# MaartenGr/ReinLife

Measured on AMD Instinct MI355X. Metric: agent-steps/sec (env.step + policy fwd), 30x30 grid, 100 agents, higher is better.
Workload: dtype f32-grade policy via block-scaled 2 x f16 split on v_mfma_f32_32x32x16_f16 (f32 accumulate) / int32+u8 world state / f64 rewards

## Files before the change

### reinlife_amd/csrc/rl_run.hip

```cpp
#include <mutex>
#include "rl_world_dev.h"
#ifndef RL_XM_DUELING_KERNEL
#define RL_XM_DUELING_KERNEL 0
#endif
#if RL_XM_DUELING_KERNEL != 0 && !defined(RL_XM_SELF_GENERATED_STATES_ONLY)
#error "RL_XM_DUELING_KERNEL != 0 is valid for self-generated states only: add -DRL_XM_SELF_GENERATED_STATES_ONLY to an A/B build that knows"
#endif
#ifndef RL_XM_ALL_DUELING_TILE
#define RL_XM_ALL_DUELING_TILE RL_XM_ALL_KERNEL
#endif
#ifndef RL_CERT_ALL
#define RL_CERT_ALL 0
#endif
#ifndef RL_XM_ALL_KERNEL
#define RL_XM_ALL_KERNEL 2
#endif

#ifdef RL_TUNING
#if !(defined(RL_RUN_UNIT) && RL_RUN_UNIT == 1)
static int g_run_debug = 0;
extern "C" __attribute__((visibility("default"))) void rl_debug_set_run_mask(int mask) { g_run_debug = mask; }
extern "C" __attribute__((visibility("default"))) int rl_debug_get_run_mask(void) { return g_run_debug; }
#endif
#define RL_RUN_DBG(ka) (*(const int __attribute__((address_space(4)))*)&(ka)->ra.debug)
static __device__ unsigned long long g_cert_counts[4];
#define RL_CERT_COUNT(greedy_mask, cert_mask, fell_back) do { \
        const unsigned long long gm_ = (greedy_mask), cm_ = (cert_mask); const bool fb_ = (fell_back); \
        if (__builtin_amdgcn_mbcnt_hi(~0u, __builtin_amdgcn_mbcnt_lo(~0u, 0u)) == 0) { \
            atomicAdd(&g_cert_counts[0], (unsigned long long)__popcll(gm_)); atomicAdd(&g_cert_counts[1], (unsigned long long)__popcll(cm_)); \
            if (fb_) atomicAdd(&g_cert_counts[2], 1ull); } } while (0)
#else
#define RL_RUN_DBG(ka) 0
#endif
#ifdef RL_TUNING
#if defined(RL_RUN_UNIT) && RL_RUN_UNIT == 1
extern "C" __attribute__((visibility("default"))) int rl_debug_cert_counters_all(unsigned long long* out)
#else
extern "C" __attribute__((visibility("default"))) int rl_debug_cert_counters(unsigned long long* out)
#endif
{
    const unsigned long long zero[4] = {0, 0, 0, 0};
    if (hipDeviceSynchronize() != hipSuccess || hipMemcpyFromSymbol(out, HIP_SYMBOL(g_cert_counts), sizeof(zero)) != hipSuccess) return -1;
    return hipMemcpyToSymbol(HIP_SYMBOL(g_cert_counts), zero, sizeof(zero)) == hipSuccess ? 0 : -1;
}
#endif

namespace {

#include "rl_policy_dev.h"

constexpr int kRunMaxBrains = 8;
constexpr int kKindAll = 4;
__host__ __device__ constexpr int kind_widest(int KIND) { return KIND == kKindAll ? RL_PPO : KIND; }

#ifndef RL_RUN_COHERENT
#define RL_RUN_COHERENT true
#endif
struct RunArgs {
    const float* packed[kRunMaxBrains];
    float eps[kRunMaxBrains];
    int kind[kRunMaxBrains];
    float* obs[2];
    int first;
    int n_ticks;
    int8_t* actions;
    const float* eps_sched;
    int eps_inline_on;
    float eps_inline[RL_EPS_INLINE_MAX];
    int trk_skip;
    int capture;
    float* policy_out;
    rl_replay rp[kRunMaxBrains];
    int debug;
};

struct PolSmem {
    short* prow;
    int* bstart;
    int* bcnt;
    int* tstart;
    short* trow;
    int* tbrain;
    int* meta;
    float* pairv;
    float* cconst;
    float* xmirror;
    int xrows;
    int xbytes;
    double* trk_scr;
    TrkLds trk;
    int* wtask;
    int* texoff;
    int* bkind;
    int* oflags;
};
constexpr int kMaxTiles = 32;
constexpr int kPairFloats = 32 + 2 * 64;
constexpr int kPairExBytes = 8 * kPlanes * 64 * 16;
constexpr int kPairFloatsAll = kPairValFloats + 2 * 64;
template <int KIND> __host__ __device__ constexpr int run_const_floats() { return KIND == kKindAll ? kTileConstMax : kTileConstFloats + kTileCertFloats; }
static_assert(kTileConstFloats + kTileCertFloats <= kTileConstMax, "kKindAll: the dueling block's value bound fits behind its constants");
template <int KIND> __host__ __device__ constexpr int run_pair_floats() { return KIND == kKindAll ? kPairFloatsAll : kPairFloats; }
template <int KIND>
__host__ __device__ inline size_t carve_policy(PolSmem& ps, char* base, size_t o, int cap, size_t mirror_budget = 0, int n_cbrains = 0,
                                               int pair_floats = run_pair_floats<KIND>(),
                                               size_t min_region = 0)
{
    o = align16(o);
    ps.xmirror = nullptr; ps.xrows = 0; ps.xbytes = 0;
    const size_t tail = 10 * (size_t)cap + 5120 + sizeof(float) * 4 * (size_t)pair_floats + sizeof(float) * run_const_floats<KIND>() * (size_t)n_cbrains;
    if (mirror_budget > o + tail) {
        const size_t rows = (mirror_budget - o - tail) / (sizeof(float) * kXStride);
        ps.xrows = (int)(rows < (size_t)cap ? rows : (size_t)cap);
        if (ps.xrows >= 32) {
            size_t bytes = sizeof(float) * kXStride * (size_t)ps.xrows;
            if (bytes < min_region && o + tail + min_region <= mirror_budget) bytes = min_region;
            ps.xmirror = (float*)(base + o); ps.xbytes = (int)bytes; o = align16(o + bytes);
        } else ps.xrows = 0;
    }
    ps.prow = (short*)(base + o); o = align16(o + sizeof(short) * (size_t)cap);
    ps.bstart = (int*)(base + o); o = align16(o + sizeof(int) * 64);
    ps.bcnt = (int*)(base + o); o = align16(o + sizeof(int) * 64);
    ps.tstart = (int*)(base + o); o = align16(o + sizeof(int) * 64);
    ps.trow = (short*)(base + o); o = align16(o + sizeof(short) * kMaxTiles * 32);
    ps.tbrain = (int*)(base + o); o = align16(o + sizeof(int) * kMaxTiles);
    ps.meta = (int*)(base + o); o = align16(o + sizeof(int) * 16);
    ps.cconst = nullptr;
    if (n_cbrains > 0) { ps.cconst = (float*)(base + o); o = align16(o + sizeof(float) * run_const_floats<KIND>() * (size_t)n_cbrains); }
    ps.pairv = nullptr;
    if (n_cbrains > 0) { ps.pairv = (float*)(base + o); o = align16(o + sizeof(float) * 4 * (size_t)pair_floats); }
    ps.wtask = (int*)(base + o); o = align16(o + sizeof(int) * 8);
    ps.texoff = (int*)(base + o); o = align16(o + sizeof(int) * 4);
    ps.bkind = (int*)(base + o); o = align16(o + sizeof(int) * kRunMaxBrains);
    if (KIND == kKindAll) { ps.oflags = (int*)(base + o); o = align16(o + sizeof(int) * 4); }
    else ps.oflags = nullptr;
    ps.trk_scr = (double*)(base + o); o = align16(o + sizeof(double) * (size_t)cap);
    ps.trk.sum = (double*)(base + o); o = align16(o + sizeof(double) * kRunMaxBrains * RL_TRK_VARS);
    ps.trk.pop = (double*)(base + o); o = align16(o + sizeof(double) * 2);
    ps.trk.cnt = (int*)(base + o); o = align16(o + sizeof(int) * kRunMaxBrains * RL_TRK_VARS);
    return o;
}
struct RunParams;
typedef const RunParams __attribute__((address_space(4))) RunParamsC;

struct RecycleRegs {
    unsigned short pos;
    int h, age, ma, g, b, u;
    uint8_t fl;
    signed char act;
    double f;
};
__device__ inline RecycleRegs recycle_read(Smem& s, int n)
{
    const int tid = rl_tidx();
    const int a = tid < n ? s.order[tid] : 0;
    RecycleRegs r;
    r.pos = s.pos[a];
    r.h = s.health[a]; r.age = s.age[a]; r.ma = s.max_age[a]; r.g = s.gene[a]; r.b = s.brain[a]; r.u = s.uid[a];
    r.fl = s.flags[a];
    r.act = s.action[a];
    r.f = s.fitness[a];
    return r;
}
#ifndef RL_SEAM_OPEN
#define RL_SEAM_OPEN 1
#endif
template <int T, bool SPEC>
__device__ __forceinline__ void recycle_world(const KParams& p, Smem& s, int n, int tick, int epoch, int next_uid, int max_gene, bool drain_stores, const RecycleRegs& rr,
                                              const int* also_drain = nullptr,
                                              bool open = false)
{
    const int tid = rl_tidx();
    const bool mine = tid < n;
    const unsigned short r_pos = rr.pos;
    const int r_h = rr.h, r_age = rr.age, r_ma = rr.ma, r_g = rr.g, r_b = rr.b, r_u = rr.u;
    const uint8_t r_fl = rr.fl;
    const signed char r_act = rr.act;
    const double r_f = rr.f;
    lds_barrier();
    if (mine) {
        s.pos[tid] = r_pos; s.health[tid] = r_h; s.age[tid] = r_age; s.max_age[tid] = r_ma; s.gene[tid] = r_g; s.brain[tid] = r_b;
        s.uid[tid] = r_u; s.flags[tid] = r_fl; s.fitness[tid] = r_f;
        if (!open) s.action[tid] = r_act;
        s.aux[tid] = 0; s.src[tid] = (short)tid; s.order[tid] = (short)tid; s.newidx[tid] = (short)tid;
        s.occ[(r_pos & 255) * p.W + (r_pos >> 8)] = (short)tid;
    }
    for (int c = tid; c < p.Cp; c += T) ((unsigned*)s.foodv)[c] = 0u;
    for (int i = tid; i < p.hash_size; i += T) { s.hkey[i] = -1; s.hcnt[i] = 0u; }
    if (tid < RL_MAX_BRAINS) s.present[tid] = 0;
    if (SPEC) for (int i = tid; i < 2 * p.cap; i += T) ((unsigned*)s.reward)[i] = 0u;
    if (tid < S_COUNT)
        s.scal[tid] = tid == S_NSLOTS ? n : tid == S_TICK ? tick : tid == S_EPOCH ? epoch : tid == S_NEXT_UID ? next_uid : tid == S_MAX_GENE ? max_gene : 0;
    const bool drain = drain_stores || (also_drain && __builtin_amdgcn_readfirstlane(*also_drain) != 0);
    if (drain) asm volatile("s_waitcnt vmcnt(0)" ::: "memory");
    if (!open || drain) lds_barrier();
}

struct RunParams {
    KParams p;
    RunArgs ra;
};
template <int TRAIN>
__device__ inline float run_eps(RunParamsC* ka, int b, int n_brains, const PolSmem& ps)
{
    typedef const float __attribute__((address_space(4))) cfloat;
    if (TRAIN) {
        if (*(const int __attribute__((address_space(4)))*)&ka->ra.eps_inline_on)
            return ((cfloat*)ka->ra.eps_inline)[__builtin_amdgcn_readfirstlane(ps.meta[3]) * n_brains + b];
        const float* es = *(const float* const __attribute__((address_space(4)))*)&ka->ra.eps_sched;
        if (es) return ((cfloat*)es)[__builtin_amdgcn_readfirstlane(ps.meta[3]) * n_brains + b];
    }
    return ((cfloat*)ka->ra.eps)[b];
}

__host__ __device__ constexpr int run_plane_stride(int T, int W, int H) { return T >= 512 ? plane_stride(W, H) : W; }
template <bool FIXED, int T>
__device__ inline KParams run_params(RunParamsC* ka)
{
#if defined(__HIP_DEVICE_COMPILE__)
    KParams p = *(const KParams __attribute__((address_space(4)))*)&ka->p;
#else
    KParams p{};
#endif
    if (FIXED) {
        p.W = kFixW; p.H = kFixH; p.C = kFixC; p.Cp = kFixCp; p.nW = kFixCp / 64; p.PS = run_plane_stride(T, kFixW, kFixH); p.invW = kFixInvW;
        p.cap = kFixCap; p.hash_size = kFixHash; p.hash_mask = kFixHash - 1;
    }
    return p;
}
constexpr size_t kRunLdsBudget = 160 * 1024;
__host__ __device__ constexpr size_t run_mirror_budget(int T) { return T >= 512 ? kRunLdsBudget : 0; }
__host__ __device__ constexpr int run_cbrains(int T, int n_brains) { return T >= 512 ? n_brains : 0; }
template <int KIND> __host__ __device__ constexpr int run_tile_floats(int T) { return T == 1024 ? kQuadFloats : run_pair_floats<KIND>(); }
__host__ __device__ constexpr size_t run_min_region(int T) { return T == 1024 ? 4 * (size_t)kQuadExBytes : 0; }
template <bool FIXED, int KIND>
__device__ inline void run_carve(const KParams& p, Smem& s, PolSmem& ps, char* smem_raw, int T)
{
    const size_t o0 = FIXED ? carve(s, smem_raw, kFixCp, kFixCap, kFixHash, plane_words(run_plane_stride(T, kFixW, kFixH), kFixH, kFixCp))
                            : carve(s, smem_raw, p.Cp, p.cap, p.hash_size, plane_words(p.PS, p.H, p.Cp));
    carve_policy<KIND>(ps, smem_raw, o0, p.cap, run_mirror_budget(T), run_cbrains(T, p.n_brains), run_tile_floats<KIND>(T), run_min_region(T));
}

template <typename F>
__device__ inline void policy_lists_wave0(const KParams& p, PolSmem& ps, int n, int lane, F brain_of)
{
    if (lane < p.n_brains) ps.bcnt[lane] = 0;
    for (int base = 0; base < n; base += 64) {
        const int k = base + lane;
        if (k < n) {
            const int b = brain_of(k);
            const int pos = __hip_atomic_fetch_add(&ps.bcnt[b], 1, __ATOMIC_RELAXED, __HIP_MEMORY_SCOPE_WORKGROUP);
            ps.prow[k] = (short)(unsigned short)(pos | (b << 10));
        }
    }
    const int mine = lane < p.n_brains ? ps.bcnt[lane] : 0;
    const int tiles = (mine + 31) >> 5;
    const int tincl = wave_incl_scan(tiles);
    const int first_tile = tincl - tiles;
    if (lane < p.n_brains) ps.tstart[lane] = first_tile;
    if (lane == 63) ps.meta[0] = tincl;
    const int tt = min(read_lane(tincl, 63), kMaxTiles);
    for (int e = lane; e < tt * 32; e += 64) ps.trow[e] = (short)0x8000;
    if (lane < tt) {
        int b = 0;
        for (int bb = 1; bb < p.n_brains; ++bb) if (read_lane(first_tile, bb) <= lane && read_lane(mine, bb) > 0) b = bb;
        ps.tbrain[lane] = b;
    }
    for (int base = 0; base < n; base += 64) {
        const int k = base + lane;
        if (k < n) {
            const int e = (unsigned short)ps.prow[k], pos = e & 1023, b = e >> 10;
            const int t = ps.tstart[b] + (pos >> 5);
            if (t < kMaxTiles) ps.trow[t * 32 + (pos & 31)] = (short)k;
        }
    }
}

__device__ inline int run_obs_flags(const KParams& p, const Smem& s, int n, int bad_health)
{
    if (bad_health || n >= 2 * p.max_agents) return 0;
    return RL_XF_SCALE | (s.type[0] == RL_AGENT ? 0 : RL_XF_INT_HEALTH);
}

__device__ inline void policy_schedule_wave0(const KParams& p, PolSmem& ps, RunParamsC* ka, int lane, bool first_call = false)
{
    const int nt = __builtin_amdgcn_readfirstlane(ps.meta[0]);
    const int t = lane & 3;
    const int brain = ps.tbrain[t] & (kRunMaxBrains - 1);
    const int kind = ps.bkind[brain];
    const int cost = t < nt ? (kind == RL_PPO ? 672 : kind == RL_DQN ? 180 : 360) : 0;
    const int ex = t < nt ? pair_ex_bytes(kind) : 0;
    int rank = 0, off = 0, total_ex = 0;
#pragma unroll
    for (int u = 0; u < 4; ++u) {
        const int cu = __builtin_amdgcn_readlane(cost, u), eu = __builtin_amdgcn_readlane(ex, u);
        rank += (cu > cost || (cu == cost && u < t)) ? 1 : 0;
        off += u < t ? eu : 0;
        total_ex += eu;
    }
    const size_t mirror_bytes = (size_t)ps.xrows * kXStride * sizeof(float);
    const bool pair_ok = nt <= 4 && ps.xmirror != nullptr && ps.pairv != nullptr && (size_t)total_ex <= mirror_bytes;
    const int fit = (int)(mirror_bytes / (size_t)pair_ex_bytes(RL_PPO));
    const int want = (0x22331100 >> (4 * (lane & 7))) & 15;
    int tile = -1, tb = 0, tk = 0;
#pragma unroll
    for (int u = 0; u < 4; ++u) {
        const int bu = __builtin_amdgcn_readlane(brain, u), ku = __builtin_amdgcn_readlane(kind, u);
        if (u < nt && __builtin_amdgcn_readlane(rank, u) == want) { tile = u; tb = bu; tk = ku; }
    }
    if (lane < 4) ps.texoff[lane] = off;
    if (lane < 8) ps.wtask[lane] = (pair_ok && tile >= 0) ? (tile | ((lane & 1) << 8) | (tb << 12) | (tk << 20)) : -1;
    if (lane == 0) {
        ps.meta[5] = pair_ok ? 0 : 1;
        if (first_call) ps.meta[6] = fit < 1 ? 1 : (fit > 4 ? 4 : fit);
    }
}

template <int T, int KIND, int TRAIN>
__device__ __forceinline__ void run_policy1(const KParams& p, Smem& s, PolSmem& ps, RunParamsC* ka, int w, int n, const float* obs_rows, char* smem_base, int wave)
{
    const int lane = rl_lane_fresh(), j = lane & 31;
    [[maybe_unused]] const int tid = wave * 64 + lane;
#ifdef RL_PHASE_PROFILE
    const long long t_entry = (long long)clock64();
#endif
    int ntiles = __builtin_amdgcn_readfirstlane(ps.meta[0]);
    {
        const int dbg = RL_RUN_DBG(ka);
        if (dbg & 4) ntiles = min(ntiles, 2);
        if (dbg & 8) ntiles = min(ntiles, 1);
        if (dbg & 16) ntiles = min(ntiles, 3);
    }
    const bool mirrored = ps.xmirror != nullptr && __builtin_amdgcn_readfirstlane(ps.meta[4]) != 0;
    [[maybe_unused]] const bool cert = T == 512 && TRAIN != 2 && !(RL_RUN_DBG(ka) & 64);
    auto tile_io = [&](int ti, TileIO& io, int j) {
        const int b = __builtin_amdgcn_readfirstlane(ps.tbrain[ti]);
        const int e = (unsigned short)ps.trow[ti * 32 + j], k = e & 0x7fff;
        io.packed = (gfloat*)((const float* const __attribute__((address_space(4)))*)ka->ra.packed)[b];
        io.obs = obs_rows;
        io.row = (int64_t)w * p.cap + k;
        io.valid = !(e & 0x8000);
        io.eps = run_eps<TRAIN>(ka, b, p.n_brains, ps);
        io.out = TRAIN == 2 ? *(float* const __attribute__((address_space(4)))*)&ka->ra.policy_out : nullptr;
        io.actions = *(int8_t* const __attribute__((address_space(4)))*)&ka->ra.actions;
        io.seed = p.seed;
        io.key_world = (uint32_t)(p.world_base + w); io.key_tick = (uint32_t)s.scal[S_TICK]; io.key_epoch = (uint32_t)s.scal[S_EPOCH];
        io.key_index = (uint32_t)k;
        io.lds_actions_off = (int)((char*)s.action - smem_base); io.lds_slot = k;
        io.x_lds_off = (mirrored && k < ps.xrows) ? (int)((char*)(ps.xmirror + k * kXStride) - smem_base) : -1;
        io.c_lds_off = ps.cconst ? (int)((char*)(ps.cconst + run_const_floats<KIND>() * b) - smem_base) : -1;
#ifdef RL_PHASE_PROFILE
        io.prof = (p.prof && (int)blockIdx.x == p.prof_world && wave == 0) ? p.prof : nullptr;
        if (io.prof && lane == 0) { io.prof[100] = t_entry; io.prof[110] = (long long)clock64(); }
#endif
    };
    if constexpr (T == 1024) {
        const int q = __builtin_amdgcn_readfirstlane(wave >> 2), slot = wave & 3;
        for (int t0 = 0; t0 < ntiles; t0 += 4) {
            const int lane = rl_lane_fresh(), j = lane & 31;
            const int ti = t0 + slot;
            const bool have = ti < ntiles;
            TileIO io;
            Tile1Part part;
            QuadLds ql;
            ql.pmax = ps.pairv + kQuadFloats * slot; ql.val = ql.pmax + 3 * 32 * 4;
            ql.ex = (f32x4*)((char*)ps.xmirror + (size_t)kQuadExBytes * slot);
#ifdef RL_PHASE_PROFILE
            ql.prof = (p.prof && (int)blockIdx.x == p.prof_world && slot == 0) ? p.prof : nullptr;
#endif
            if (have) {
                tile_io(ti, io, j);
                if (ntiles > 4) io.x_lds_off = -1;
                policy_quad<KIND, RL_RUN_COHERENT>(io, lane, q, &ql, &part);
            } else {
#pragma unroll
                for (int i = 0; i < kQuadBarriers; ++i) lds_barrier();
            }
            lds_barrier();
            if (have && q == 0) tile1_finish<KIND>(io, lane, part.head, ql.val[j], part.draw, *(const f32x4*)((const float*)(smem_base + io.c_lds_off) + 768 + 8 + 4 * (lane >> 5)));
        }
    } else
    if (T == 512 && !cert && ps.pairv != nullptr && ntiles <= 4 && (size_t)ps.xrows * kXStride * sizeof(float) >= 4 * (size_t)kPairExBytes) {
        const int role = __builtin_amdgcn_readfirstlane(wave >> 2), slot = wave & 3;
        const bool have = slot < ntiles;
        TileIO io;
        Tile1Part part;
        PairLds pl;
        pl.val = ps.pairv + kPairFloats * slot; pl.pmax = pl.val + 32;
        pl.ex = (f32x4*)((char*)ps.xmirror + (size_t)kPairExBytes * slot);
        if (have) {
            tile_io(slot, io, j);
            policy_tile1s<KIND, RL_RUN_COHERENT, true, RL_XM_DUELING_KERNEL>(io, lane, role, &pl, &part);
        } else { lds_barrier(); lds_barrier(); }
#ifdef RL_PHASE_PROFILE
        if (p.prof && (int)blockIdx.x == p.prof_world && lane == 0) p.prof[116 + wave] = (long long)clock64();
#endif
        lds_barrier();
        if (have && role == 0) {
            const int fl = rl_lane_fresh();
            tile1_finish<KIND>(io, fl, part.head, pl.val[fl & 31], part.draw, *(const f32x4*)((const float*)(smem_base + io.c_lds_off) + 768 + 8 + 4 * (fl >> 5)));
        }
    } else {
        for (int ti = wave; ti < ntiles; ti += T / 64) {
            TileIO io;
            tile_io(ti, io, j);
            if (T == 512 && cert) policy_tile1s<KIND, RL_RUN_COHERENT, false, RL_XM_DUELING_KERNEL, T == 512 && TRAIN != 2>(io, lane);
            else if (T == 512) policy_tile1s<KIND, RL_RUN_COHERENT, false, RL_XM_DUELING_KERNEL>(io, lane);
            else policy_tile1<KIND, RL_RUN_COHERENT, true>(io, lane);
        }
#ifdef RL_PHASE_PROFILE
        if (T == 512 && p.prof && (int)blockIdx.x == p.prof_world && lane == 0) p.prof[116 + wave] = (long long)clock64();
#endif
    }
#ifdef RL_PHASE_PROFILE
    if (p.prof && (int)blockIdx.x == p.prof_world && tid == 0) p.prof[111] = (long long)clock64();
#endif
    lds_barrier();
#ifdef RL_PHASE_PROFILE
    if (p.prof && (int)blockIdx.x == p.prof_world && tid == 0) p.prof[112] = (long long)clock64();
#endif
}

#ifndef RL_XM_COLD_CALL
#define RL_XM_COLD_CALL 0
#endif
#ifndef RL_XM_LIKELY
#define RL_XM_LIKELY 1
#endif
#if RL_XM_LIKELY
#define RL_XM_EXPECT(x) __builtin_expect_with_probability(!!(x), 1, 0.9)
#else
#define RL_XM_EXPECT(x) (x)
#endif
template <bool CERT>
__device__ __attribute__((noinline, cold)) Tile1Part run_tile_general(TileIO io, PairLds pl, int role, int kind)
{
    Tile1Part part;
    const int lane = rl_lane_fresh();
    if (kind == RL_DQN) policy_pair2<RL_DQN, RL_RUN_COHERENT>(io, lane, role, &pl, &part);
    else if (kind == RL_PPO) policy_pair2<RL_PPO, RL_RUN_COHERENT>(io, lane, role, &pl, &part);
    else policy_tile1s<RL_PERD3QN, RL_RUN_COHERENT, true, 0, CERT>(io, lane, role, &pl, &part);
    return part;
}

template <int T, int TRAIN>
__device__ __forceinline__ void run_policy_all(const KParams& p, Smem& s, PolSmem& ps, RunParamsC* ka, int w, int n, const float* obs_rows, char* smem_base, int wave)
{
    static_assert(T == 512, "kKindAll: 512-thread workgroups");
    typedef const int __attribute__((address_space(4))) cint;
    const int lane = rl_lane_fresh(), j = lane & 31;
#ifdef RL_PHASE_PROFILE
    if (p.prof && (int)blockIdx.x == p.prof_world && wave == 0 && lane == 0) p.prof[100] = (long long)clock64();
#endif
    const int ntiles = __builtin_amdgcn_readfirstlane(ps.meta[0]);
    const bool mirrored = ps.xmirror != nullptr && __builtin_amdgcn_readfirstlane(ps.meta[4]) != 0;
    const bool fallback = __builtin_amdgcn_readfirstlane(ps.meta[5]) != 0;
    constexpr int xneed = RL_XM_ALL_KERNEL == 2 ? (RL_XF_SCALE | RL_XF_INT_HEALTH) : RL_XF_SCALE;
#ifdef RL_XM_ASSUME_ALWAYS
    const bool rows_known = true;
#else
    const bool rows_known = RL_XM_ALL_KERNEL != 0 && (__builtin_amdgcn_readfirstlane(ps.oflags[0]) & xneed) == xneed;
#endif
    auto tile_io = [&](int ti, TileIO& io, bool from_mirror, int task) {
        const int b = task >= 0 ? ((task >> 12) & 255) : __builtin_amdgcn_readfirstlane(ps.tbrain[ti]);
        const int e = (unsigned short)ps.trow[ti * 32 + j], k = e & 0x7fff;
        io.packed = (gfloat*)((const float* const __attribute__((address_space(4)))*)ka->ra.packed)[b];
        io.obs = obs_rows;
        io.row = (int64_t)w * p.cap + k;
        io.valid = !(e & 0x8000);
        io.eps = run_eps<TRAIN>(ka, b, p.n_brains, ps);
        io.out = TRAIN == 2 ? *(float* const __attribute__((address_space(4)))*)&ka->ra.policy_out : nullptr;
        io.actions = *(int8_t* const __attribute__((address_space(4)))*)&ka->ra.actions;
        io.seed = p.seed;
        io.key_world = (uint32_t)(p.world_base + w); io.key_tick = (uint32_t)s.scal[S_TICK]; io.key_epoch = (uint32_t)s.scal[S_EPOCH];
        io.key_index = (uint32_t)k;
        io.lds_actions_off = (int)((char*)s.action - smem_base); io.lds_slot = k;
        io.x_lds_off = (from_mirror && mirrored && k < ps.xrows) ? (int)((char*)(ps.xmirror + k * kXStride) - smem_base) : -1;
        io.c_lds_off = (int)((char*)(ps.cconst + kTileConstMax * b) - smem_base);
#ifdef RL_PHASE_PROFILE
        io.prof = (p.prof && (int)blockIdx.x == p.prof_world && wave == ((p.ablate >> 20) & 7)) ? p.prof : nullptr;
#endif
        return task >= 0 ? ((task >> 20) & 7) : ((cint*)ka->ra.kind)[b];
// ... 17 lines not shown
            else if (RL_XM_EXPECT(rows_known)) {
                if (kind == RL_DQN) policy_pair2<RL_DQN, RL_RUN_COHERENT, RL_XM_ALL_KERNEL>(io, lane, role, &pl, &part);
                else if (kind == RL_PPO) policy_pair2<RL_PPO, RL_RUN_COHERENT, RL_XM_ALL_KERNEL>(io, lane, role, &pl, &part);
                else duel(IntC<RL_XM_ALL_DUELING_TILE>{}, io, role, pl, part);
            } else if (RL_XM_COLD_CALL) part = cert ? run_tile_general<TRAIN != 2>(io, pl, role, kind) : run_tile_general<false>(io, pl, role, kind);
            else {
                if (kind == RL_DQN) policy_pair2<RL_DQN, RL_RUN_COHERENT>(io, lane, role, &pl, &part);
                else if (kind == RL_PPO) policy_pair2<RL_PPO, RL_RUN_COHERENT>(io, lane, role, &pl, &part);
                else duel(IntC<0>{}, io, role, pl, part);
            }
        } else { lds_barrier(); lds_barrier(); }
        lds_barrier();
        if (have && role == 0) {
            const int fl = rl_lane_fresh();
            if (kind == RL_DQN) pair_finish<RL_DQN>(io, fl, part, &pl);
            else if (kind == RL_PPO) pair_finish<RL_PPO>(io, fl, part, &pl);
            else if (!cert) tile1_finish<RL_PERD3QN>(io, fl, part.head, pl.val[fl & 31], part.draw, *(const f32x4*)((const float*)(smem_base + io.c_lds_off) + 768 + 8 + 4 * (fl >> 5)));
        }
    };
    const int pr = __builtin_amdgcn_readfirstlane(ps.meta[6]);
    const int task = __builtin_amdgcn_readfirstlane(ps.wtask[wave]);
    const int n_rounds = fallback ? (ntiles + pr - 1) / pr : 1;
    for (int r = 0; r < n_rounds; ++r) {
        const int slot = fallback ? (wave & 3) : (task & 255);
        const int ti = fallback ? r * pr + slot : slot;
        const bool have = fallback ? (slot < pr && ti < ntiles) : task >= 0;
        const int role = __builtin_amdgcn_readfirstlane(fallback ? (wave >> 2) : ((task >> 8) & 1));
        const int ex_off = fallback ? slot * pair_ex_bytes(RL_PPO) : (have ? ps.texoff[slot] : 0);
        pair_round(have, ti, role, slot, ex_off, !fallback, fallback ? -1 : task);
        if (fallback) lds_barrier();
    }
#ifdef RL_PHASE_PROFILE
    if (p.prof && (int)blockIdx.x == p.prof_world && lane == 0) p.prof[116 + wave] = (long long)clock64();
    if (p.prof && (int)blockIdx.x == p.prof_world && wave == 0 && lane == 0) p.prof[111] = (long long)clock64();
#endif
    lds_barrier();
#ifdef RL_PHASE_PROFILE
    if (p.prof && (int)blockIdx.x == p.prof_world && wave == 0 && lane == 0) p.prof[112] = (long long)clock64();
#endif
}

template <int T, bool FIXED, int KIND, int TRAIN>
__device__ __forceinline__ void run_policy_half(RunParamsC* ka, int wave)
{
    extern __shared__ __attribute__((aligned(16))) char smem_raw[];
    const KParams p = run_params<FIXED, T>(ka);
    Smem s;
    PolSmem ps;
    run_carve<FIXED, KIND>(p, s, ps, smem_raw, T);
    const int w = blockIdx.x;
    const int n = __builtin_amdgcn_readfirstlane(ps.meta[1]), cur = __builtin_amdgcn_readfirstlane(ps.meta[2]);
    const float* obs_in = ((float* const __attribute__((address_space(4)))*)ka->ra.obs)[cur];
    if constexpr (KIND == kKindAll) run_policy_all<T, TRAIN>(p, s, ps, ka, w, n, obs_in, smem_raw, wave);
    else run_policy1<T, KIND, TRAIN>(p, s, ps, ka, w, n, obs_in, smem_raw, wave);
}

template <int T>
__device__ inline void patch_planes_after_update(const KParams& p, Smem& s, int n1, int first_new, int end_new)
{
    const int tid = rl_tidx();
    bool cell0 = false;
    for (int k = tid; k < n1; k += T) {
        const int a = s.order[k];
        const int fl = s.flags[a], ps = s.pos[a];
        if (fl & RL_F_DEAD) {
            const int c = (ps & 255) * p.PS + (ps >> 8);
            s.foodv[c] = 0.5f; s.healthv[c] = -1.f; s.genev[c] = -2;
            cell0 |= c == 0;
        }
    }
    for (int i = first_new + tid; i < end_new; i += T) {
        const int c = cell_to_plane(p, s.tgt[i]);
        s.foodv[c] = 0.f; s.healthv[c] = 1.f; s.genev[c] = -2;
        cell0 |= c == 0;
    }
    if (cell0) s.scal[S_PLANES_DIRTY] = 1;
}

__device__ inline rl_replay load_replay(RunParamsC* ka, int b)
{
#if defined(__HIP_DEVICE_COMPILE__)
    return *(const rl_replay __attribute__((address_space(4)))*)&ka->ra.rp[b];
#else
    return rl_replay{};
#endif
}
__device__ inline void capture_reserve(const KParams& p, Smem& s, RunParamsC* ka, int n1, int* slot)
{
    const int lane = lane_id();
    int cnt = 0;
    for (int base = 0; base < n1; base += 64) {
        const int k = base + lane;
        const int a = k < n1 ? s.order[k] : 0;
        const int br = (k < n1 && s.age[a] > 1) ? s.brain[a] : -1;
        for (int bb = 0; bb < p.n_brains; ++bb) { const int c = __popcll(__ballot(br == bb)); if (lane == bb) cnt += c; }
    }
    unsigned long long pos = 0, capacity = 1;
    if (lane < p.n_brains) {
        const rl_replay R = load_replay(ka, lane);
        capacity = (unsigned long long)R.capacity;
        if (cnt) pos = atomicAdd(R.count, (unsigned long long)cnt);
    }
    for (int base = 0; base < n1; base += 64) {
        const int k = base + lane;
        const int a = k < n1 ? s.order[k] : 0;
        const int br = (k < n1 && s.age[a] > 1) ? s.brain[a] : -1;
        int mine = -1;
        for (int bb = 0; bb < p.n_brains; ++bb) {
            const unsigned long long m = __ballot(br == bb);
            const unsigned long long start = read_lane_u64(pos, bb), capb = read_lane_u64(capacity, bb);
            if (br == bb) mine = (int)((start + (unsigned long long)__popcll(m & lowmask(lane))) % capb);
            if (lane == bb) pos += (unsigned long long)__popcll(m);
        }
        if (k < n1) slot[k] = mine;
    }
}
template <int T>
__device__ __forceinline__ void capture_rows(const KParams& p, Smem& s, RunParamsC* ka, int w, int n1, const int* slot, const float* state_rows)
{
    const int t = rl_tidx();
    constexpr int G = T / 49;
    const int g0 = t / 49, idx = t - g0 * 49;
    const int dr = idx / 7 - 3, dc = idx - (idx / 7) * 7 - 3;
    const __amdgpu_buffer_rsrc_t rsrc = __builtin_amdgcn_make_buffer_rsrc((void*)state_rows, 0, 0x7fffffff, 0x00027000);
    auto ld = [&](int64_t float_index) { return __builtin_bit_cast(float, __builtin_amdgcn_raw_buffer_load_b32(rsrc, (int)(float_index * 4), 0, 16 )); };
    const int64_t wbase = (int64_t)w * p.cap;
    if (g0 < G)
        for (int k = g0; k < n1; k += G) {
            const int sl = slot[k];
            if (sl < 0) continue;
            const int a = s.order[k];
            const rl_replay R = load_replay(ka, s.brain[a]);
            const int pa = s.pos[a];
            int ci = (pa & 255) + dr, cj = (pa >> 8) + dc;
            ci += ci < 0 ? p.H : 0; ci -= ci >= p.H ? p.H : 0;
            cj += cj < 0 ? p.W : 0; cj -= cj >= p.W ? p.W : 0;
            const int c = ci * p.PS + cj;
            const int g = s.genev[c];
            float* d1 = R.state_prime + (size_t)sl * RL_OBS_DIM + idx;
            d1[0] = s.foodv[c]; d1[49] = s.healthv[c]; d1[98] = g == -2 ? 0.f : (g == s.gene[a] ? 1.f : -1.f);
            const int64_t src = (wbase + a) * RL_OBS_DIM + idx;
            float* d0 = R.state + (size_t)sl * RL_OBS_DIM + idx;
            d0[0] = ld(src); d0[49] = ld(src + 49); d0[98] = ld(src + 98);
        }
    float* const pout = *(float* const __attribute__((address_space(4)))*)&ka->ra.policy_out;
    for (int k = t; k < n1; k += T) {
        const int sl = slot[k];
        if (sl < 0) continue;
        const int a = s.order[k];
        const rl_replay R = load_replay(ka, s.brain[a]);
        const int same = (int)(s.hcnt[s.hslot[a]] >> 16);
        float* d1 = R.state_prime + (size_t)sl * RL_OBS_DIM + 147;
        d1[0] = (float)((double)s.health[a] * rl_one_200th());
        d1[1] = (s.flags[a] & RL_F_REPRODUCED) ? 1.f : 0.f;
        d1[2] = (float)((double)same / (double)n1);
        d1[3] = (float)((double)n1 / (double)p.max_agents);
        d1[4] = (s.flags[a] & RL_F_KILLED) ? 1.f : 0.f;
        d1[5] = (s.flags[a] & RL_F_ATE_SUPER) ? 1.f : -1.f;
        const int64_t src = (wbase + a) * RL_OBS_DIM + 147;
        float* d0 = R.state + (size_t)sl * RL_OBS_DIM + 147;
#pragma unroll
        for (int e = 0; e < 6; ++e) d0[e] = ld(src + e);
        const int act = s.action[a];
        R.action[sl] = (int8_t)act;
        R.reward[sl] = (float)s.reward[a];
        R.done[sl] = (s.flags[a] & RL_F_DEAD) ? 1 : 0;
        R.age[sl] = s.age[a];
        if (pout && R.prob && act >= 0 && act < 8) {
            const __amdgpu_buffer_rsrc_t rq = __builtin_amdgcn_make_buffer_rsrc((void*)pout, 0, 0x7fffffff, 0x00027000);
            R.prob[sl] = __builtin_bit_cast(float, __builtin_amdgcn_raw_buffer_load_b32(rq, (int)(((wbase + a) * 8 + act) * 4), 0, 16));
        }
    }
}

template <int T, bool FIXED, int KIND, int TRAIN>
__device__ __forceinline__ void run_tick_body(RunParamsC* ka)
{
    extern __shared__ __attribute__((aligned(16))) char smem_raw[];
    const KParams p = run_params<FIXED, T>(ka);
    Smem s;
    PolSmem ps;
    run_carve<FIXED, KIND>(p, s, ps, smem_raw, T);
    const int w = blockIdx.x;
    const int n0 = __builtin_amdgcn_readfirstlane(ps.meta[1]), cur = __builtin_amdgcn_readfirstlane(ps.meta[2]);
    const int ticks_done = __builtin_amdgcn_readfirstlane(ps.meta[3]);
    float* const obs_out = ((float* const __attribute__((address_space(4)))*)ka->ra.obs)[cur ^ 1];
    const int tid = rl_tidx();
    constexpr bool kSpec = T == 1024;
    int nslots = n0;
    constexpr bool kPlanesEarly = T >= 256;
    RL_MARK(60);
    phase_step<T, true, kPlanesEarly, kSpec>(p, s, w, n0);
    RL_MARK(61);
    assign_order<T>(p, s, nslots);
    if (kPlanesEarly) patch_placed_planes(p, s);
    const int n1 = s.scal[S_N1];
    lds_barrier();
    RL_MARK(62);
    const bool overlapped = !p.limit_reproduction;
    const size_t b = (size_t)w * p.cap;
    auto step_outputs = [&](int t, int nt) {
        for (int k = t; k < n1; k += nt) {
            const int a = s.order[k];
            if (p.so.reward) p.so.reward[b + k] = (float)s.reward[a];
            if (p.so.done) p.so.done[b + k] = (s.flags[a] & RL_F_DEAD) ? 1 : 0;
            if (p.so.src) p.so.src[b + k] = (short)a;
        }
        if (t == 0 && p.so.n_acted) p.so.n_acted[w] = n0;
        if (t == 0 && p.so.acted_total && n0) atomicAdd(p.so.acted_total, (unsigned long long)n0);
    };
    const bool trk = TRAIN && T >= 256 && p.so.trk_tick != nullptr;
    const bool cap = TRAIN == 2 && T >= 256 && *(const int __attribute__((address_space(4)))*)&ka->ra.capture != 0;
    int* const cap_slot = (int*)ps.trk_scr;
    auto track = [&]() {
        if (trk) track_world_wave0(p, s, w, n1, ps.trk_scr, &ps.trk, ticks_done >= *(const int __attribute__((address_space(4)))*)&ka->ra.trk_skip);
        if (cap) capture_reserve(p, s, ka, n1, cap_slot);
    };
    if (overlapped) {
        if (tid < 64) {
            if (!p.static_families) best_agents_wave(s, n1);
            reproduce_wave0<T, true>(p, s, w, n1, nslots);
        } else if (TRAIN && (trk || cap)) {
            if (tid < 128) track();
            else {
                write_observations<(T >= 256 ? T - 128 : 64)>(p, s, w, n1, p.so.obs, tid - 128);
                step_outputs(tid - 128, T - 128);
            }
        } else {
            write_observations<(T > 64 ? T - 64 : 64)>(p, s, w, n1, p.so.obs, tid - 64);
            step_outputs(tid - 64, T - 64);
        }
    } else if (TRAIN && (trk || cap)) {
        if (tid >= 64 && tid < 128) track();
        else {
            const int t = tid < 64 ? tid : tid - 64;
            write_observations<(T >= 256 ? T - 64 : 64)>(p, s, w, n1, p.so.obs, t);
            step_outputs(t, T - 64);
        }
    } else {
        write_observations<T>(p, s, w, n1, p.so.obs);
        step_outputs(tid, T);
    }
    lds_barrier();
    RL_MARK(63);
    if (TRAIN == 2 && cap) {
        capture_rows<T>(p, s, ka, w, n1, cap_slot, ((float* const __attribute__((address_space(4)))*)ka->ra.obs)[cur]);
        lds_barrier();
    }
    for (int a = tid; a < nslots; a += T) s.src[a] = s.newidx[a];
    if (!overlapped) lds_barrier();
    else { const int first_new = nslots; nslots = s.scal[S_NSLOTS]; patch_planes_after_update<T>(p, s, n1, first_new, nslots); }
    if (!overlapped) phase_update<T, true>(p, s, w, n1, nslots, true);
    if (tid >= T - 64) {
        const int l = tid - (T - 64);
        unsigned long long mine = 0ull;
        for (int wd = 0; wd < p.nW; ++wd) {
            const unsigned long long m = __ballot(s.type[wd * 64 + l] == RL_AGENT);
            if (l == wd) mine = m;
        }
        const int cntw = __popcll(mine);
        const int incl = wave_incl_scan(cntw);
        s.agbits[l] = mine;
        s.wordbase[l] = incl - cntw;
        if (l == 63) s.scal[S_N2] = incl;
    }
    static_assert(T > 64, "k_run: at least two waves");
    if (tid < T - 64)
        for (int i = tid; i < p.hash_size; i += T - 64) { s.hkey[i] = -1; s.hcnt[i] = 0u; }
    lds_barrier();
    RL_MARK(64);
    RL_MARK(65);
    int n2 = s.scal[S_N2];
    int tick_next = s.scal[S_TICK] + 1, epoch_next = s.scal[S_EPOCH];
    int next_uid = s.scal[S_NEXT_UID], max_gene = s.scal[S_MAX_GENE];
    const bool refill = p.refill_threshold >= 0 && n2 < p.refill_threshold;
    if (refill) {
        const bool prepared = kSpec && s.scal[S_SPEC_DONE] != 0;
        const uint32_t new_epoch = (uint32_t)epoch_next + 1u;
        if (prepared) {
            n2 = apply_spec_refill<T>(p, s, w, new_epoch);
            const int np2 = (n2 + 63) & ~63;
            for (int k = tid; k < np2; k += T) hash_insert_wave(s, p.hash_mask, k < n2, k, k < n2 ? s.gene[k] : 0, 1u << 16);
        } else {
            n2 = reset_world_lds<T>(p, s, w, new_epoch);
            rebuild_gene_counts<T>(p, s, n2);
        }
        tick_next = 0; epoch_next = (int)new_epoch; next_uid = n2; max_gene = p.n_brains;
    } else {
        assign_order<T>(p, s, nslots);
        const int nsp = (nslots + 63) & ~63;
        for (int a = tid; a < nsp; a += T) {
            const int aa = a < nslots ? a : 0;
            const int ps_ = s.pos[aa], ge = s.gene[aa];
            const bool on = a < nslots && s.occ[(ps_ & 255) * p.W + (ps_ >> 8)] == a;
            hash_insert_wave(s, p.hash_mask, on, a, on ? ge : 0, 1u << 16);
        }
    }
    RL_MARK(66);
    if (refill || !overlapped || s.scal[S_PLANES_DIRTY]) build_planes<T>(p, s);
    lds_barrier();
    RL_MARK(67);
    if (p.uo.src)
        for (int k = tid; k < n2; k += T) p.uo.src[b + k] = refill ? (short)-1 : s.src[s.order[k]];
    const RecycleRegs rr = recycle_read(s, n2);
    {
        if (tid < 64) {
            policy_lists_wave0(p, ps, n2, tid, [&](int k) { return s.brain[s.order[k]]; });
            if (T == 1024 && tid == 0) ps.meta[5] = ps.meta[0] > 4;
            RL_MARK_T(96, 0);
            if constexpr (KIND == kKindAll) policy_schedule_wave0(p, ps, ka, tid);
            RL_MARK_T(97, 0);
        } else {
            if constexpr (KIND == kKindAll) { if (tid == 64) ps.oflags[0] = run_obs_flags(p, s, n2, ps.oflags[1]); }
            write_observations<(T > 64 ? T - 64 : 64)>(p, s, w, n2, obs_out, tid - 64, ps.xmirror, ps.xrows);
            RL_MARK_T(98, 64); RL_MARK_T(99, T - 64);
        }
    }
    RL_MARK(68);
    if (tid == 0) { ps.meta[1] = n2; ps.meta[2] = cur ^ 1; ps.meta[3] = ticks_done + 1; }
    if (ticks_done == 0 && tid == 0) ps.meta[4] = ps.xmirror != nullptr;
    if (RL_SEAM_OPEN && tid == 64) { s.scal[S_TICK] = tick_next; s.scal[S_EPOCH] = epoch_next; }
    const bool seam_open = RL_SEAM_OPEN && T == 512 && ticks_done + 1 < *(const int __attribute__((address_space(4)))*)&ka->ra.n_ticks;
    recycle_world<T, kSpec>(p, s, n2, tick_next, epoch_next, next_uid, max_gene, ps.xmirror == nullptr || n2 > ps.xrows || (TRAIN == 2 && cap), rr,
                            (KIND == kKindAll || T == 1024) ? &ps.meta[5] : nullptr,
                            seam_open);
    RL_MARK(69);
}

template <int T, int KIND, int TRAIN>
__device__ __forceinline__ void run_tick_call_fixed(RunParamsC* ka) { run_tick_body<T, true, KIND, TRAIN>(ka); }
template <int T, int KIND, int TRAIN>
__device__ __forceinline__ void run_tick_call_generic(RunParamsC* ka) { run_tick_body<T, false, KIND, TRAIN>(ka); }

template <int KIND>
__device__ inline void run_cert_bounds(const KParams& p, PolSmem& ps, RunParamsC* ka, int tid)
{
    typedef const int __attribute__((address_space(4))) cint;
    constexpr int CF = run_const_floats<KIND>();
    const int nb = p.n_brains, wave = tid >> 6;
    auto dueling = [&](int b) { return KIND != kKindAll || ((cint*)ka->ra.kind)[b] == RL_D3QN || ((cint*)ka->ra.kind)[b] == RL_PERD3QN; };
    double* part = (double*)ps.pairv;
    for (int b0 = 0; b0 < nb; b0 += 2) {
        double c[2][2];
#pragma unroll
        for (int i = 0; i < 2; ++i) {
            const int b = b0 + i;
            c[i][0] = 0.0; c[i][1] = 0.0;
            if (b < nb && dueling(b)) cert_bound_part((gfloat*)((const float* const __attribute__((address_space(4)))*)ka->ra.packed)[b], tid, c[i][0], c[i][1]);
        }
#pragma unroll
        for (int off = 32; off >= 1; off >>= 1)
#pragma unroll
            for (int i = 0; i < 2; ++i) { c[i][0] += __shfl_xor(c[i][0], off); c[i][1] += __shfl_xor(c[i][1], off); }
        if ((tid & 63) == 0) {
#pragma unroll
            for (int i = 0; i < 2; ++i)
                if (b0 + i < nb) { part[((b0 + i) * 8 + wave) * 2] = c[i][0]; part[((b0 + i) * 8 + wave) * 2 + 1] = c[i][1]; }
        }
    }
    lds_barrier();
    if (tid < nb && dueling(tid)) {
        double c0 = 0.0, c1 = 0.0;
        for (int w = 0; w < 8; ++w) { c0 += part[(tid * 8 + w) * 2]; c1 += part[(tid * 8 + w) * 2 + 1]; }
        float* const k = ps.cconst + CF * tid;
        k[kTileConstFloats] = f32_up(((double)fabsf(k[768 + 16 + 8]) + c0) * (1.0 + 0x1p-8));
        k[kTileConstFloats + 1] = f32_up(c1 * (1.0 + 0x1p-8));
    }
}

template <int T, bool FIXED, int KIND, int TRAIN>
__device__ __forceinline__ void run_load_call(RunParamsC* ka)
{
    extern __shared__ __attribute__((aligned(16))) char smem_raw[];
    typedef const int __attribute__((address_space(4))) cint;
    const KParams p = run_params<FIXED, T>(ka);
    Smem s;
    PolSmem ps;
    run_carve<FIXED, KIND>(p, s, ps, smem_raw, T);
    int n0;
    RL_MARK(90);
    const int tid = rl_tidx();
    const int first = *(cint*)&ka->ra.first;
    const int n_pre = ((cint*)ka->p.st.n_agents)[blockIdx.x];
    const bool preload = ps.xmirror != nullptr && n_pre <= ps.xrows;
    constexpr int NT = T > 64 ? T - 64 : T;
    const int pt = T > 64 ? tid - 64 : tid;
    typedef const f32x4 __attribute__((address_space(1))) gvec;
    gvec* rows4 = (gvec*)(((float* const __attribute__((address_space(4)))*)ka->ra.obs)[first] + (size_t)blockIdx.x * p.cap * RL_OBS_DIM);
    const int total = n_pre * RL_OBS_DIM, nvec = (total + 3) >> 2;
    constexpr int U = 8, UC = 4;
    f32x4 rv[U];
    float cv[UC];
    if (preload && pt >= 0 && nvec > 0) {
#pragma unroll
        for (int u = 0; u < U; ++u) rv[u] = rows4[min(u * NT + pt, nvec - 1)];
    }
    constexpr int CF = run_const_floats<KIND>();
    const int ctotal = ps.cconst ? CF * p.n_brains : 0;
    auto const_src = [&](int i) -> gfloat* {
        const int b = i / CF, j = i - CF * b;
        gfloat* pk = (gfloat*)((const float* const __attribute__((address_space(4)))*)ka->ra.packed)[b];
        if constexpr (KIND == kKindAll) {
            const int kind = ((const int __attribute__((address_space(4)))*)ka->ra.kind)[b];
            return pk + tile_const_src(kind, min(j, tile_const_floats(kind) - 1));
        } else
            return pk + tile_const_src(KIND, min(j, kTileConstFloats - 1));
    };
    if (ctotal > 0) {
#pragma unroll
        for (int u = 0; u < UC; ++u) cv[u] = *const_src(min(u * T + tid, ctotal - 1));
    }
    load_world<T, (T == 1024)>(p, s, (int)blockIdx.x, n0);
    RL_MARK(91);
    auto put_rows = [&](int q, const f32x4& v) {
        if (q < nvec) {
#pragma unroll
            for (int e = 0; e < 4; ++e) {
                const int i = 4 * q + e, r = i / RL_OBS_DIM;
                if (i < total) ps.xmirror[r * kXStride + (i - r * RL_OBS_DIM)] = v[e];
            }
        }
    };
    if (preload && pt >= 0 && nvec > 0) {
#pragma unroll
        for (int u = 0; u < U; ++u) put_rows(u * NT + pt, rv[u]);
        for (int base = NT * U; base < nvec; base += NT * U) {
#pragma unroll
            for (int u = 0; u < U; ++u) rv[u] = rows4[min(base + u * NT + pt, nvec - 1)];
#pragma unroll
            for (int u = 0; u < U; ++u) put_rows(base + u * NT + pt, rv[u]);
        }
    }
    if (preload && pt >= 0)
        for (int r = pt; r < n_pre; r += NT) {
            float* m = ps.xmirror + r * kXStride + 153;
            m[0] = 0.0f; m[1] = 0.0f; m[2] = 0.0f; *(float4*)(m + 3) = float4{0.0f, 0.0f, 0.0f, 0.0f};
        }
    RL_MARK(92);
    if constexpr (KIND == kKindAll) {
        int bad = 0;
        for (int a = tid; a < n0; a += T) bad |= (s.health[a] >= 400 || s.health[a] <= -400) ? 1 : 0;
        bad = __any(bad);
        if (tid == 0) ps.oflags[1] = 0;
        lds_barrier();
        if (bad && (tid & 63) == 0) ps.oflags[1] = 1;
        lds_barrier();
    }
    if (tid == 0) {
        ps.meta[1] = n0; ps.meta[2] = first; ps.meta[3] = 0; ps.meta[4] = preload ? 1 : 0;
        if constexpr (KIND == kKindAll) ps.oflags[0] = run_obs_flags(p, s, n0, ps.oflags[1]);
    }
    if (TRAIN && p.so.trk_tick) {
        const int G = p.static_families ? p.n_brains : 1, t = tid;
        const size_t o = (size_t)blockIdx.x * G * RL_TRK_VARS;
        if (t < G * RL_TRK_VARS) { ps.trk.sum[t] = p.so.trk_sum[o + t]; ps.trk.cnt[t] = p.so.trk_cnt[o + t]; }
        if (t < 2) ps.trk.pop[t] = p.so.trk_pop[(size_t)blockIdx.x * 3 + 1 + t];
    }
    if (tid < 64) {
        if constexpr (KIND == kKindAll) { if (tid < kRunMaxBrains) ps.bkind[tid] = tid < p.n_brains ? ((const int __attribute__((address_space(4)))*)ka->ra.kind)[tid] : RL_D3QN; }
        policy_lists_wave0(p, ps, n0, tid, [&](int k) { return s.brain[k]; });
        if (T == 1024 && tid == 0) ps.meta[5] = ps.meta[0] > 4;
        if constexpr (KIND == kKindAll) policy_schedule_wave0(p, ps, ka, tid, true);
    }
    RL_MARK(93);
    if (ctotal > 0) {
#pragma unroll
        for (int u = 0; u < UC; ++u) { const int i = u * T + tid; if (i < ctotal) ps.cconst[i] = cv[u]; }
        for (int base = T * UC; base < ctotal; base += T * UC) {
#pragma unroll
            for (int u = 0; u < UC; ++u) cv[u] = *const_src(min(base + u * T + tid, ctotal - 1));
#pragma unroll
            for (int u = 0; u < UC; ++u) { const int i = base + u * T + tid; if (i < ctotal) ps.cconst[i] = cv[u]; }
        }
        if constexpr (T == 512 && (KIND != kKindAll || RL_CERT_ALL)) run_cert_bounds<KIND>(p, ps, ka, tid);
    }
    RL_MARK(94);
    lds_barrier();
    RL_MARK(95);
}
template <int T, bool FIXED, int KIND, int TRAIN>
__device__ __forceinline__ void run_store_call(RunParamsC* ka)
{
    extern __shared__ __attribute__((aligned(16))) char smem_raw[];
    const KParams p = run_params<FIXED, T>(ka);
    Smem s;
    PolSmem ps;
    run_carve<FIXED, KIND>(p, s, ps, smem_raw, T);
    store_world<T>(p, s, (int)blockIdx.x, ps.meta[1]);
    if (TRAIN && p.so.trk_tick) {
        const int G = p.static_families ? p.n_brains : 1, t = rl_tidx();
        const size_t o = (size_t)blockIdx.x * G * RL_TRK_VARS;
        if (t < G * RL_TRK_VARS) { p.so.trk_sum[o + t] = ps.trk.sum[t]; p.so.trk_cnt[o + t] = ps.trk.cnt[t]; }
        if (t < 2) p.so.trk_pop[(size_t)blockIdx.x * 3 + 1 + t] = ps.trk.pop[t];
    }
    if (rl_tidx() == 0) { p.st.tick[blockIdx.x] = s.scal[S_TICK]; p.st.epoch[blockIdx.x] = s.scal[S_EPOCH]; p.st.next_uid[blockIdx.x] = s.scal[S_NEXT_UID]; p.st.max_gene[blockIdx.x] = s.scal[S_MAX_GENE]; }
}

template <int T, bool FIXED, int KIND, int TRAIN>
__global__ __launch_bounds__(T) void k_run(const RunParams rp)
{
    RunParamsC* ka = (RunParamsC*)__builtin_amdgcn_kernarg_segment_ptr();
    typedef const int __attribute__((address_space(4))) cint;
    const int n_ticks = *(cint*)&ka->ra.n_ticks;
    const int dbg = RL_RUN_DBG(ka);
#ifdef RL_PHASE_PROFILE
#define RL_KMARK(i) do { long long* pf_ = *(long long* const __attribute__((address_space(4)))*)&ka->p.prof; \
        if (pf_ && (int)blockIdx.x == *(cint*)&ka->p.prof_world && threadIdx.x == 0) RL_G(pf_)[i] = (long long)clock64(); } while (0)
#else
#define RL_KMARK(i) do { } while (0)
#endif
    RL_KMARK(70);
#ifndef RL_STAGGER_BEFORE_LOAD
    const long long t_entry = (long long)clock64();
    run_load_call<T, FIXED, KIND, TRAIN>(ka);
    RL_KMARK(71);
    if (!(dbg & 32)) {
        const long long until = t_entry + (long long)(blockIdx.x & 15) * 500;
        while ((long long)clock64() < until) __builtin_amdgcn_s_sleep(2);
    }
#else
    if (!(dbg & 32)) {
        const long long until = (long long)clock64() + (long long)(blockIdx.x & 15) * 500;
        while ((long long)clock64() < until) __builtin_amdgcn_s_sleep(2);
    }
    RL_KMARK(71);
    run_load_call<T, FIXED, KIND, TRAIN>(ka);
#endif
    RL_KMARK(72);
    const int wave = __builtin_amdgcn_readfirstlane((int)threadIdx.x >> 6);
    for (int it = 0; it < n_ticks; ++it) {
        if (!(dbg & 1)) run_policy_half<T, FIXED, KIND, TRAIN>(ka, wave);
        if (it == 0) RL_KMARK(73);
        if (!(dbg & 2)) {
            if constexpr (FIXED) run_tick_call_fixed<T, KIND, TRAIN>(ka);
            else run_tick_call_generic<T, KIND, TRAIN>(ka);
        }
        if (it == 0) RL_KMARK(74);
        if (it == 1) RL_KMARK(75);
    }
    RL_KMARK(76);
    run_store_call<T, FIXED, KIND, TRAIN>(ka);
    asm volatile("s_waitcnt vmcnt(0)" ::: "memory");
    RL_KMARK(77);
}

}

#if defined(RL_RUN_UNIT) && RL_RUN_UNIT == 1
const void* rl_run_fn_all(int fixed, int train)
{
#define RL_RUN_ALL(FX, TR) if (fixed == (FX ? 1 : 0) && train == TR) return (const void*)k_run<512, FX, kKindAll, TR>;
    RL_RUN_ALL(true, 0) RL_RUN_ALL(true, 1) RL_RUN_ALL(true, 2) RL_RUN_ALL(false, 0) RL_RUN_ALL(false, 1) RL_RUN_ALL(false, 2)
#undef RL_RUN_ALL
    return nullptr;
}
#else
#if defined(RL_RUN_UNIT)
const void* rl_run_fn_all(int fixed, int train);
#endif

static int run_kind_of(const rl_brain* brains, int n_brains)
{
    if (n_brains < 1 || n_brains > kRunMaxBrains) return -1;
    bool duel = true;
    for (int b = 0; b < n_brains; ++b) {
        if (brains[b].kind < RL_DQN || brains[b].kind > RL_PPO) return -1;
        duel = duel && (brains[b].kind == RL_D3QN || brains[b].kind == RL_PERD3QN);
    }
    return duel ? RL_PERD3QN : kKindAll;
}
template <int KIND>
static size_t run_smem_bytes(const rl_world* h, int T, int stride, int* xrows = nullptr, size_t* xbytes = nullptr)
{
    PolSmem ps;
    const size_t world = rl_world_smem_bytes(h->cpad, h->cfg.slot_cap, h->hash_size, stride, h->cfg.height);
    const size_t b = carve_policy<KIND>(ps, nullptr, world, h->cfg.slot_cap, run_mirror_budget(T), run_cbrains(T, h->cfg.n_brains), run_tile_floats<KIND>(T), run_min_region(T));
    if (xrows) *xrows = ps.xrows;
    if (xbytes) *xbytes = (size_t)ps.xbytes;
    return b;
}
template <int KIND>
static int host_plane_stride(const rl_world* h, int T)
{
    const int padded = run_plane_stride(T, h->cfg.width, h->cfg.height);
    return (padded != h->cfg.width && run_smem_bytes<KIND>(h, T, padded) > 160 * 1024) ? h->cfg.width : padded;
}
static int run_block(const rl_world* h)
{
    const int forced = h->opt.world_block;
    if (forced == 256 || forced == 512 || forced == 1024) return forced;
    if (h->cfg.n_worlds <= 768) return 512;
#ifdef RL_RUN_256
    return 256;
#else
    return h->opt.run_always ? 512 : 256;
#endif
}
static bool has_perdqn(const rl_brain* brains, int n_brains)
{
    for (int b = 0; b < n_brains; ++b)
        if (brains[b].kind == RL_PERDQN) return true;
    return false;
}
int rl_world_run_supported(const rl_world* h, const rl_brain* brains, int n_brains)
{
    if (has_perdqn(brains, n_brains)) {
        rl_set_error("rl_run: PERDQN brains are not run by the multi-tick kernel: use the two-launch loop (rl_policy_act + rl_tick_refill)");
        return 0;
    }
    const int kind = run_kind_of(brains, n_brains);
    if (kind < 0) return 0;
    const int T = run_block(h);
    if (h->cfg.slot_cap > T) return 0;
#ifndef RL_RUN_1024
    if (T == 1024) { rl_set_error("rl_run: 1024-thread workgroups are a tuning-build instantiation (-DRL_RUN_1024), not in this library"); return 0; }
#endif
#ifndef RL_RUN_256
    if (T == 256) { rl_set_error("rl_run: 256-thread workgroups are a tuning-build instantiation (-DRL_RUN_256), not in this library"); return 0; }
#endif
    if (kind == kKindAll) {
        if (T != 512) return 0;
        int xrows = 0;
        if (run_smem_bytes<kKindAll>(h, T, host_plane_stride<kKindAll>(h, T), &xrows) > 160 * 1024) return 0;
        return (size_t)xrows * kXStride * sizeof(float) >= (size_t)pair_ex_bytes(RL_PPO);
    }
// ... 95 lines not shown
```

Before: 1.102 billion.

## Split seam recycle work onto upper waves so lower waves return early

At the tick seam in the 512-thread, non-all-kind, non-training path, the world recycle (agent compaction, occupancy, food, hash and scalar reset) is now done only by waves 4-7, which read recycle entries offset by half the block. Waves 0-3 return immediately, skipping the barrier and drain, so they can move on to the next tick's policy work sooner. The split applies only when the observation mirror covers all rows and more ticks remain. The trade-off is that half as many threads do the reset loops, and correctness now relies on the later barrier ordering these LDS writes before the next reads.

Measured after the change: 1.100 billion. Within noise of the previous version (-0.2%).

```diff
diff --git a/reinlife_amd/csrc/rl_run.hip b/reinlife_amd/csrc/rl_run.hip
--- a/reinlife_amd/csrc/rl_run.hip
+++ b/reinlife_amd/csrc/rl_run.hip
@@ -143,6 +143,7 @@
 struct RunParams;
 typedef const RunParams __attribute__((address_space(4))) RunParamsC;
 
+constexpr int kSeamMirrorRowsMax = 160 * 1024 / (4 * kXStride);
 struct RecycleRegs {
     unsigned short pos;
     int h, age, ma, g, b, u;
@@ -162,13 +163,29 @@
     r.f = s.fitness[a];
     return r;
 }
+__device__ inline RecycleRegs recycle_read_entry(Smem& s, int n, int k)
+{
+    const int a = k < n ? s.order[k] : 0;
+    RecycleRegs r;
+    r.pos = s.pos[a];
+    r.h = s.health[a]; r.age = s.age[a]; r.ma = s.max_age[a]; r.g = s.gene[a]; r.b = s.brain[a]; r.u = s.uid[a];
+    r.fl = s.flags[a];
+    r.act = s.action[a];
+    r.f = s.fitness[a];
+    return r;
+}
 #ifndef RL_SEAM_OPEN
 #define RL_SEAM_OPEN 1
 #endif
-template <int T, bool SPEC>
+#ifndef RL_SEAM_JOBS
+#define RL_SEAM_JOBS 1
+#endif
+__host__ __device__ constexpr bool seam_jobs(int T, int KIND, int TRAIN) { return RL_SEAM_JOBS != 0 && RL_SEAM_OPEN && T == 512 && KIND != kKindAll && TRAIN != 2; }
+template <int T, bool SPEC, bool JOBS = false>
 __device__ __forceinline__ void recycle_world(const KParams& p, Smem& s, int n, int tick, int epoch, int next_uid, int max_gene, bool drain_stores, const RecycleRegs& rr,
                                               const int* also_drain = nullptr,
-                                              bool open = false)
+                                              bool open = false,
+                                              bool split = false)
 {
     const int tid = rl_tidx();
     const bool mine = tid < n;
@@ -178,6 +195,26 @@
     const signed char r_act = rr.act;
     const double r_f = rr.f;
     lds_barrier();
+    if constexpr (JOBS) {
+        if (split) {
+            static_assert(T == 512 && !SPEC, "the seam's jobs: waves 4-7 of eight");
+            static_assert(kSeamMirrorRowsMax < T / 2, "split: every row mirrored, one slot per thread of waves 4-7");
+            if (__builtin_amdgcn_readfirstlane(tid >> 6) < 4) return;
+            const int t = tid - T / 2;
+            if (t < n) {
+                s.pos[t] = r_pos; s.health[t] = r_h; s.age[t] = r_age; s.max_age[t] = r_ma; s.gene[t] = r_g; s.brain[t] = r_b;
+                s.uid[t] = r_u; s.flags[t] = r_fl; s.fitness[t] = r_f;
+                s.aux[t] = 0; s.src[t] = (short)t; s.order[t] = (short)t; s.newidx[t] = (short)t;
+                s.occ[(r_pos & 255) * p.W + (r_pos >> 8)] = (short)t;
+            }
+            for (int c = t; c < p.Cp; c += T / 2) ((unsigned*)s.foodv)[c] = 0u;
+            for (int i = t; i < p.hash_size; i += T / 2) { s.hkey[i] = -1; s.hcnt[i] = 0u; }
+            if (t < RL_MAX_BRAINS) s.present[t] = 0;
+            if (t < S_COUNT)
+                s.scal[t] = t == S_NSLOTS ? n : t == S_TICK ? tick : t == S_EPOCH ? epoch : t == S_NEXT_UID ? next_uid : t == S_MAX_GENE ? max_gene : 0;
+            return;
+        }
+    }
     if (mine) {
         s.pos[tid] = r_pos; s.health[tid] = r_h; s.age[tid] = r_age; s.max_age[tid] = r_ma; s.gene[tid] = r_g; s.brain[tid] = r_b;
         s.uid[tid] = r_u; s.flags[tid] = r_fl; s.fitness[tid] = r_f;
@@ -801,7 +838,14 @@
     RL_MARK(67);
     if (p.uo.src)
         for (int k = tid; k < n2; k += T) p.uo.src[b + k] = refill ? (short)-1 : s.src[s.order[k]];
-    const RecycleRegs rr = recycle_read(s, n2);
+    constexpr bool kJobs = seam_jobs(T, KIND, TRAIN);
+    [[maybe_unused]] bool split = false;
+    [[maybe_unused]] int tid_entry = tid;
+    if constexpr (kJobs) {
+        split = ticks_done + 1 < *(const int __attribute__((address_space(4)))*)&ka->ra.n_ticks && ps.xmirror != nullptr && n2 <= ps.xrows && !(RL_RUN_DBG(ka) & 1);
+        if (split) tid_entry = tid >= T / 2 ? tid - T / 2 : n2;
+    }
+    const RecycleRegs rr = kJobs ? recycle_read_entry(s, n2, tid_entry) : recycle_read(s, n2);
     {
         if (tid < 64) {
             policy_lists_wave0(p, ps, n2, tid, [&](int k) { return s.brain[s.order[k]]; });
@@ -820,6 +864,9 @@
     if (ticks_done == 0 && tid == 0) ps.meta[4] = ps.xmirror != nullptr;
     if (RL_SEAM_OPEN && tid == 64) { s.scal[S_TICK] = tick_next; s.scal[S_EPOCH] = epoch_next; }
     const bool seam_open = RL_SEAM_OPEN && T == 512 && ticks_done + 1 < *(const int __attribute__((address_space(4)))*)&ka->ra.n_ticks;
+    if constexpr (kJobs)
+        recycle_world<T, kSpec, true>(p, s, n2, tick_next, epoch_next, next_uid, max_gene, ps.xmirror == nullptr || n2 > ps.xrows, rr, nullptr, seam_open, split);
+    else
     recycle_world<T, kSpec>(p, s, n2, tick_next, epoch_next, next_uid, max_gene, ps.xmirror == nullptr || n2 > ps.xrows || (TRAIN == 2 && cap), rr,
                             (KIND == kKindAll || T == 1024) ? &ps.meta[5] : nullptr,
                             seam_open);
```
